# KLab/YAIK

Measured on AMD Instinct MI355X. Metric: Mpix/s tile encode (alpha reject + 7 gradient passes + 8x8 range quant), 8K RGBA, higher is better.
Workload: dtype u8/int32 (+f32 mode-selection sums)

## Files before the change

### yaik_amd/csrc/yk_api.hip

```cpp
#include "yk_common.h"
#ifdef YK_TEST_HOOKS
#include "../../include/yaik_hip_test.h"
#endif
#include <cstdio>
#include <cstring>
#include <utility>
#include <vector>

int yk_fail(yk_ctx* c, int code, const char* what, hipError_t e) {
    if (c && c->err.empty()) {
        c->err = what ? what : "error";
        if (e != hipSuccess) { c->err += ": "; c->err += hipGetErrorString(e); }
    }
    return code;
}

int yk_refuse(yk_ctx* c, int code, const char* what) {
    if (c) c->err = what ? what : "error";
    return code;
}

void yk_rebase(yk_ctx* c, int f) {
    const YkFrameStrides& fs = c->fs; auto& B = c->B;
    c->curFrame = f;
    for (int i = 0; i < 4; i++) c->plane[i] = B.plane[i] ? B.plane[i] + (size_t)f * fs.plane : nullptr;
    c->keep = B.keep + (size_t)f * fs.keep; c->bounds = B.bounds + (size_t)f * 16;
    for (int i = 0; i < 7; i++) c->bitmap[i] = B.bitmap[i] + (size_t)f * fs.bitmap[i];
    c->coverage = B.coverage + (size_t)f * fs.coverage; c->tileDef = B.tileDef + (size_t)f * fs.tileDef;
    c->tileCount = B.tileCount + (size_t)f * fs.tileCount; c->slots = B.slots + (size_t)f * fs.slots;
    c->blockSums = B.blockSums + (size_t)f * fs.blockN; c->blockCnt = B.blockCnt + (size_t)f * fs.blockN;
    c->totals = B.totals + (size_t)f * 8; c->defsOut = B.defsOut + (size_t)f * fs.defsOut; c->nibOut = B.nibOut + (size_t)f * fs.nibOut;
}

static void yk_input_changed(yk_ctx* c) {
    c->encoded = false; c->alphaDone = false; c->alphaFinished = false; c->avBatchValid = false; c->img.sb.valid = false; c->pal.valid = false;
    c->cornersReady = false; c->ppActive = false; c->ppLastBit = 0; c->previewFresh = false;
}

static void yk_encode_done(yk_ctx* c, int wantDst) {
    c->encoded = true; c->dstValid = wantDst != 0; c->img.sb.valid = false; c->pal.valid = false; c->cornersReady = false; c->ppActive = false;
    c->ppLastBit = 0; c->previewFresh = false; c->nextCornerPass = 0; c->r1Ready = false;
}

static void yk_free_image(yk_ctx* c) {
    c->img = YkImageBufs();
    { yk_ctx::Bases none = {}; for (int i = 0; i < 4; i++) none.plane[i] = c->B.plane[i]; c->B = none; }
    c->keep = nullptr; c->bounds = nullptr; for (int i = 0; i < 7; i++) c->bitmap[i] = nullptr;
    c->coverage = nullptr; c->tileDef = nullptr; c->tileCount = nullptr; c->slots = nullptr;
    c->blockSums = nullptr; c->blockCnt = nullptr; c->totals = nullptr; c->defsOut = nullptr; c->nibOut = nullptr;
    c->ppBitmapBytes = c->ppStreamBytes = 0; c->r1Ready = false; c->pixCacheValid = false;
    if (c->frameGraph) { (void)hipGraphExecDestroy(c->frameGraph); c->frameGraph = nullptr; }
    yk_input_changed(c);
}

static int yk_alloc_image_run(yk_ctx* c) {
    const size_t F = (size_t)c->nFrames;
    const size_t T8 = (size_t)c->tilesW * c->tilesH, MT = (size_t)c->mtW * c->mtH;
    auto& B = c->B; auto& M = c->img; YkFrameStrides& fs = c->fs; const hipStream_t s = c->stream;
    auto up = [](size_t n, size_t a) { return (n + a - 1) / a * a; };
    fs.keep = up(MT + 4, 16);
    YK_HIP(c, M.keep.alloc(s, fs.keep * F, 16));
    YK_HIP(c, M.bounds.alloc(s, 16 * F));
    {
        const size_t nUnits = (size_t)((c->fullW / 4 + 63) / 64) * c->mtH, nGroups = (nUnits + 63) / 64;
        YK_HIP(c, M.alphaUnitBox.alloc(s, (nUnits + nGroups) * F * 4, 16));
        YK_HIP(c, M.alphaArrive.alloc(s, (nGroups + 1) * F, 16));
        YK_HIP(c, hipMemset(M.alphaArrive, 0, (nGroups + 1) * F * sizeof(uint32_t) + 16));
    }
    static const int sh[7][2] = { {4,4},{4,3},{3,4},{3,3},{3,2},{2,3},{2,2} };
    size_t cur = 0, oBm[7], oBm0b, oCov, oInfo, oRun;
    auto place = [&](size_t bytesPerFrame) { const size_t o = cur; cur = up(cur + bytesPerFrame * F + 16, 256); return o; };
    for (int i = 0; i < 7; i++) {
        const int bx = (sh[i][0] == 2) ? 32 : 64, by = (sh[i][1] == 2) ? 32 : 64;
        const size_t bits = (size_t)((c->fullW + bx - 1) / bx) * ((c->h + by - 1) / by) * ((bx >> sh[i][0]) * (by >> sh[i][1]));
        c->bitmapBytes[i] = bits >> 3;
        fs.bitmap[i] = up(c->bitmapBytes[i] + 4, 16);
        oBm[i] = place(fs.bitmap[i]);
    }
    const size_t nB64 = (size_t)((c->fullW + 63) / 64) * ((c->h + 63) / 64);
    fs.bm0b = up(nB64 * 4, 16); oBm0b = place(fs.bm0b);
    fs.coverage = up(MT, 8); oCov = place(fs.coverage * sizeof(uint16_t));
    fs.tileInfo = up(T8, 2); oInfo = place(fs.tileInfo * sizeof(uint2));
    fs.runSums = up((T8 + 7) / 8, 4); oRun = place(fs.runSums * sizeof(uint32_t));
    if (cur >= ((size_t)1 << 32)) return yk_fail(c, YK_ERR_BAD_ARG, "image too large for 32-bit offsets into the small-output arena");
    YK_HIP(c, M.small.alloc(s, cur));
    YK_HIP(c, hipMemset(M.small, 0, cur));
    B.small = M.small;
    for (int i = 0; i < 7; i++) B.bitmap[i] = B.small + oBm[i];
    B.bm0b = B.small + oBm0b; B.coverage = reinterpret_cast<uint16_t*>(B.small + oCov);
    B.tileInfo = reinterpret_cast<uint2*>(B.small + oInfo); B.runSums = reinterpret_cast<uint32_t*>(B.small + oRun);
    fs.tileDef = 3 * T8; fs.tileCount = 3 * T8; fs.slots = 3 * T8 * YK_SLOT;
    YK_HIP(c, M.tileDef.alloc(s, fs.tileDef * F, 16));
    YK_HIP(c, M.tileCount.alloc(s, fs.tileCount * F, 16));
    YK_HIP(c, M.slots.alloc(s, fs.slots * F, 16));
    c->nScanBlocks = (int)((T8 + 1023) / 1024);
    fs.blockN = (size_t)c->nScanBlocks * 2;
    YK_HIP(c, M.blockSums.alloc(s, fs.blockN * F));
    YK_HIP(c, M.blockCnt.alloc(s, fs.blockN * F));
    YK_HIP(c, hipMemset(M.blockCnt, 0, fs.blockN * F * sizeof(uint32_t)));
    YK_HIP(c, M.totals.alloc(s, 8 * F));
    fs.defsOut = 3 * T8;
    YK_HIP(c, M.defsOut.alloc(s, fs.defsOut * F, 16));
    c->nibStride = T8 * YK_SLOT + 64;
    fs.nibOut = 3 * c->nibStride;
    YK_HIP(c, M.nibOut.alloc(s, fs.nibOut * F, 16));
    B.keep = M.keep; B.bounds = M.bounds; B.tileDef = M.tileDef; B.tileCount = M.tileCount; B.slots = M.slots;
    B.blockSums = M.blockSums; B.blockCnt = M.blockCnt; B.totals = M.totals; B.defsOut = M.defsOut; B.nibOut = M.nibOut;
    c->dstValid = false;
    yk_rebase(c, 0);
    return YK_OK;
}
static int yk_alloc_image(yk_ctx* c) {
    const int rc = yk_alloc_image_run(c);
    if (rc) yk_free_image(c);
    return rc;
}

static int yk_stage_fold(yk_ctx* c, int st) {
    for (int k = 0; k < c->stN[st]; k++) {
        float t = 0;
        YK_HIP(c, hipEventSynchronize(c->stEv[st][k][1]));
// ... 760 lines not shown
```

### yaik_amd/csrc/yk_common.h

```cpp
#pragma once
#include <hip/hip_runtime.h>
#include <stdint.h>
#include <stddef.h>
#include <memory>
#include <string>
#include <vector>
#include "../../include/yaik_hip.h"

#define YK_BLK      64
#define YK_LSTRIDE  68
#define YK_LROWS    65
#define YK_EV_RING  64
#define YK_SLOT     32
#define YK_NUM_STAGES 11
#define YK_STAGE_RING 16

struct YkFrameStrides {
    unsigned long long plane, keep, bitmap[7], coverage, tileDef, tileCount, slots, blockN, defsOut, nibOut;
    unsigned long long bm0b, tileInfo, runSums;
};

enum { YK_EVSET_ALPHA = 1, YK_EVSET_PACK = 2 };
enum { YK_EV_A0, YK_EV_E0, YK_EV_E1, YK_EV_P1, YK_EV_N };
struct YkEvRing {
// ... 34 lines not shown
    int ablate;
    const uint8_t* keep;
    const int32_t* bounds;
    uint8_t* bitmap[7];
    uint16_t* coverage;
    uint16_t* tileDef;
    uint8_t*  tileCount;
    uint8_t*  slots;
    uint32_t* blockCnt;
    int32_t*  dst[3];
    int tilesW, tilesH, mtW, mtH;
    int xBB64, yBB64, xBB32, yBB32;
    int nFrames;
    const uint8_t* qtab;
    uint8_t* small;
    uint32_t oBm[7], oBm0b, oCov, oInfo, oRun;
    uint4* pixCache;
    YkFrameStrides fs;
};

#define YK_SB_COUNTS 9
struct YkStreamRec { uint8_t* rgb[7]; uint8_t* pix; uint8_t* type; };
struct YkStreamsBatch {
    YkBuf<uint32_t> owner;
    YkBuf<uint32_t> cScratch;
    YkBuf<uint32_t> r1Scratch;
    YkBuf<uint32_t> counts;
    YkBuf<uint8_t> out;
    YkBuf<YkStreamRec> tab;
    std::vector<yk_frame_streams> table; bool valid = false;
    int what = 0;
};

struct YkPalette {
    YkBuf<uint8_t> scratch;
    YkBuf<uint8_t> out;
    YkBuf<uint32_t> carry;
    bool carryFresh = true;
    std::vector<uint8_t> segHost;
    std::vector<uint32_t> lenBase;
    int nSeg = 0; bool valid = false;
};

struct YkPaletteDec {
    YkBuf<uint8_t> scratch;
    YkBuf<uint8_t> out;
    YkBuf<uint8_t> stage;
    std::vector<size_t> slotOff, slotLen;
    std::vector<uint32_t> statusHost;
    size_t statusOff = 0;
    int nSeg = 0; bool valid = false;
};

struct YkImageBufs {
    YkBuf<uint8_t> keep; YkBuf<int32_t> bounds;
    YkBuf<int> alphaUnitBox;
    YkBuf<uint32_t> alphaArrive;
    YkBuf<uint8_t> small;
    YkBuf<uint16_t> tileDef; YkBuf<uint8_t> tileCount, slots;
    YkBuf<int32_t> dst[3];
    YkBuf<uint32_t> blockSums, blockCnt, totals;
    YkBuf<unsigned long long> exportSizes;
    YkBuf<uint16_t> defsOut; YkBuf<uint8_t> nibOut;
    YkBuf<uint32_t> latticeOwner; YkBuf<uint8_t> cornerStream; YkBuf<uint32_t> cornerScratch;
    YkBuf<uint32_t> cornerEdgeIdx;
    YkBuf<uint16_t> covCh;
    YkBuf<uint8_t> mapped3;
    YkBuf<uint32_t> ppBitmap; YkBuf<uint8_t> ppStream; YkBuf<uint32_t> ppScratch;
    YkBuf<int32_t> preview;
    YkBuf<uint8_t> r1Slots, r1Params; YkBuf<uint32_t> r1Cnt; YkBuf<uint8_t> r1Pix, r1Type;
    YkBuf<uint4> pixCache;
    YkStreamsBatch sb;
};

struct yk_ctx {
    int device = -1;
    int numCU = 256;
    const uint8_t* qtab = nullptr;
    hipStream_t ownStream = nullptr;
    hipStream_t stream = nullptr;
    std::string err;
    int fullW = 0, fullH = 0, nPlanes = 0, y0 = 0, h = 0, halo = 0;
    int tilesW = 0, tilesH = 0, mtW = 0, mtH = 0;
    int nFrames = 1, curFrame = 0;
    YkFrameStrides fs = {};
    struct Bases {
        const int32_t* plane[4]; uint8_t* keep; int32_t* bounds; uint8_t* bitmap[7]; uint16_t* coverage; uint16_t* tileDef; uint8_t* tileCount;
        uint8_t* slots; uint32_t* blockSums; uint32_t* blockCnt; uint32_t* totals; uint16_t* defsOut; uint8_t* nibOut;
        uint8_t* small;
        uint8_t* bm0b; uint2* tileInfo; uint32_t* runSums;
    } B = {};
    const int32_t* plane[4] = {nullptr, nullptr, nullptr, nullptr};
    int strideElems = 0;
    YkBuf<int32_t> ownedPlanes;
    YkBuf<uint8_t> pxStage;
    hipEvent_t evPixCopy = nullptr;
    uint8_t* keep = nullptr;
    int32_t* bounds = nullptr;
    int boundsOff = 8;
    bool alphaDone = false, alphaFinished = false;
    int32_t hostBounds[4] = {0, 0, 0, 0}; int hostDiscard = 1, hostHasChunk = 0;
    uint8_t* bitmap[7] = {}; size_t bitmapBytes[7] = {};
    uint16_t* coverage = nullptr;
    uint16_t* tileDef = nullptr; uint8_t* tileCount = nullptr; uint8_t* slots = nullptr;
    int32_t dstFill = -1; bool dstValid = false;
    uint32_t* blockSums = nullptr;
    uint32_t* blockCnt = nullptr;
    uint32_t* totals = nullptr;
    hipEvent_t evHandoff = nullptr;
    hipEvent_t fusedAfter = nullptr; std::shared_ptr<YkEvRing> fusedAfterRing;
// ... 94 lines not shown
```

### yaik_amd/csrc/yk_stages.hip

```cpp
#include "yk_common.h"
#ifdef YK_TEST_HOOKS
#include "../../include/yaik_hip_test.h"
#endif
#include "yk_device.h"

typedef int yk_i4 __attribute__((ext_vector_type(4)));
#ifndef YK_ALPHA_THREADS
#define YK_ALPHA_THREADS 256
#endif
#define YK_ALPHA_WAVES (YK_ALPHA_THREADS / 64)
#ifndef YK_ALPHA_ROWS
#define YK_ALPHA_ROWS 2
#endif
__global__ __launch_bounds__(YK_ALPHA_THREADS) void yk_alpha_kernel(const int32_t* __restrict__ alpha0, int strideElems, int w, int h, int y0,
                                                       uint8_t* __restrict__ keep0, int mtW, int mtH, int32_t* __restrict__ bounds,
                                                       int nFrames, unsigned long long planeStride, unsigned long long keepStride,
                                                       int* __restrict__ unitBox0, uint32_t* __restrict__ arrive0) {
    __shared__ int s_box[YK_ALPHA_WAVES][4];
    const int lane = threadIdx.x & 63, wv = threadIdx.x >> 6;
    const int vecPerRow = w >> 2;
    const int nSeg = (vecPerRow + YK_ALPHA_THREADS - 1) / YK_ALPHA_THREADS;
    const int nRowUnits = (mtH + YK_ALPHA_ROWS - 1) / YK_ALPHA_ROWS;
    const int nUnits = nSeg * nRowUnits, nGroups = (nUnits + 63) >> 6;
    for (long long uu = blockIdx.x; uu < (long long)nUnits * nFrames; uu += gridDim.x) {
        const int f = (int)(uu / nUnits), u = (int)(uu - (long long)f * nUnits);
        const int32_t* alpha = alpha0 + (size_t)f * planeStride;
        uint8_t* keep = keep0 + (size_t)f * keepStride;
        int* unitBox = unitBox0 + (size_t)f * (nUnits + nGroups) * 4;
        uint32_t* arrive = arrive0 + (size_t)f * (nGroups + 1);
        const int tyU = u / nSeg, seg = u - tyU * nSeg;
        const int xv = seg * YK_ALPHA_THREADS + (int)threadIdx.x;
        const bool inX = xv < vecPerRow;
        const bool tileLane = (lane & 3) == 0;
        const int tx = xv >> 2;
        int colLo = 0x7FFFFFFF, colHi = -1, rowLo = 0x7FFFFFFF, rowHi = -1;
        const int xvc = min(xv, vecPerRow - 1);
        int nzR[YK_ALPHA_ROWS];
        bool und[YK_ALPHA_ROWS];
        {
            yk_i4 p[YK_ALPHA_ROWS][2];
#pragma unroll
            for (int r = 0; r < YK_ALPHA_ROWS; r++) {
                const int yA = min((tyU * YK_ALPHA_ROWS + r) * 16, h - 1), yB = min(yA + 15, h - 1);
                p[r][0] = __builtin_nontemporal_load(reinterpret_cast<const yk_i4*>(alpha + (size_t)yA * strideElems + (size_t)xvc * 4));
                p[r][1] = __builtin_nontemporal_load(reinterpret_cast<const yk_i4*>(alpha + (size_t)yB * strideElems + (size_t)xvc * 4));
            }
            bool anyUnd = false;
#pragma unroll
            for (int r = 0; r < YK_ALPHA_ROWS; r++) {
                const bool on = inX && (tyU * YK_ALPHA_ROWS + r) * 16 < h;
                const yk_i4 o = p[r][0] | p[r][1];
                nzR[r] = on ? (o.x | o.y | o.z | o.w) : 0;
                const unsigned long long pb = __ballot(nzR[r] != 0);
                und[r] = on && ((pb >> (lane & ~3)) & 0xFULL) == 0;
                anyUnd |= und[r];
            }
            if (__ballot(anyUnd) != 0) {
                yk_i4 a[YK_ALPHA_ROWS][14];
#pragma unroll
                for (int r = 0; r < YK_ALPHA_ROWS; r++) {
                    const int ty = tyU * YK_ALPHA_ROWS + r;
                    const int32_t* col = alpha + (size_t)(ty * 16) * strideElems + (size_t)xv * 4;
#pragma unroll
                    for (int k = 0; k < 14; k++) {
                        a[r][k] = (yk_i4){0, 0, 0, 0};
                        if (und[r] && ty * 16 + 1 + k < h) a[r][k] = __builtin_nontemporal_load(reinterpret_cast<const yk_i4*>(col + (size_t)(1 + k) * strideElems));
                    }
                }
#pragma unroll
                for (int r = 0; r < YK_ALPHA_ROWS; r++)
#pragma unroll
                    for (int k = 0; k < 14; k++) nzR[r] |= a[r][k].x | a[r][k].y | a[r][k].z | a[r][k].w;
            }
        }
#pragma unroll
        for (int r = 0; r < YK_ALPHA_ROWS; r++) {
            const int ty = tyU * YK_ALPHA_ROWS + r;
            if (ty >= mtH) break;
            const int nz = nzR[r];
            const unsigned long long b = __ballot(nz != 0);
            const bool kept = ((b >> (lane & ~3)) & 0xFULL) != 0;
            if (tileLane && tx < mtW) keep[(size_t)ty * mtW + tx] = kept ? 1 : 0;
            const unsigned long long kb64 = __ballot(tileLane && kept && tx < mtW);
            if (kb64) {
                const int t0 = seg * (YK_ALPHA_THREADS / 4) + wv * 16;
                colLo = min(colLo, t0 + ((__ffsll((long long)kb64) - 1) >> 2));
                colHi = max(colHi, t0 + ((63 - __clzll((long long)kb64)) >> 2));
                rowLo = min(rowLo, ty); rowHi = max(rowHi, ty);
            }
        }
        if (lane == 0) { s_box[wv][0] = colLo; s_box[wv][1] = colHi; s_box[wv][2] = rowLo; s_box[wv][3] = rowHi; }
        __syncthreads();
        if (wv == 0) {
            unsigned long long* ub = reinterpret_cast<unsigned long long*>(unitBox);
            auto putBox = [&](const int slot, const int bx0, const int by0, const int bx1, const int by1) {
                __hip_atomic_store(&ub[slot * 2], ((unsigned long long)(uint32_t)by0 << 32) | (uint32_t)bx0, __ATOMIC_RELAXED, __HIP_MEMORY_SCOPE_AGENT);
                __hip_atomic_store(&ub[slot * 2 + 1], ((unsigned long long)(uint32_t)by1 << 32) | (uint32_t)bx1, __ATOMIC_RELAXED, __HIP_MEMORY_SCOPE_AGENT);
                __builtin_amdgcn_s_waitcnt(0);
            };
            auto foldBoxes = [&](const int first, const int n, int& x0, int& gy0, int& x1, int& gy1) {
                x0 = 9999999; gy0 = 9999999; x1 = -1; gy1 = -1;
                for (int k = lane; k < n; k += 64) {
                    const unsigned long long a = __hip_atomic_load(&ub[(first + k) * 2], __ATOMIC_RELAXED, __HIP_MEMORY_SCOPE_AGENT);
                    const unsigned long long bb = __hip_atomic_load(&ub[(first + k) * 2 + 1], __ATOMIC_RELAXED, __HIP_MEMORY_SCOPE_AGENT);
                    x0 = min(x0, (int)(uint32_t)a); gy0 = min(gy0, (int)(uint32_t)(a >> 32)); x1 = max(x1, (int)(uint32_t)bb); gy1 = max(gy1, (int)(uint32_t)(bb >> 32));
                }
#pragma unroll
                for (int d = 1; d < 64; d <<= 1) {
                    x0 = min(x0, __shfl_xor(x0, d)); x1 = max(x1, __shfl_xor(x1, d));
                    gy0 = min(gy0, __shfl_xor(gy0, d)); gy1 = max(gy1, __shfl_xor(gy1, d));
                }
            };
            const int g = u >> 6, inGroup = min(64, nUnits - (g << 6));
            uint32_t lastOfGroup = 0;
            if (lane == 0) {
                int lo = s_box[0][0], hi = s_box[0][1], rlo = s_box[0][2], rhi = s_box[0][3];
#pragma unroll
                for (int k = 1; k < YK_ALPHA_WAVES; k++) { lo = min(lo, s_box[k][0]); hi = max(hi, s_box[k][1]); rlo = min(rlo, s_box[k][2]); rhi = max(rhi, s_box[k][3]); }
                const bool any = hi >= 0;
                putBox(u, any ? lo * 16 : 9999999, any ? y0 + rlo * 16 : 9999999, any ? hi * 16 + 16 : -1, any ? y0 + rhi * 16 + 16 : -1);
                lastOfGroup = __hip_atomic_fetch_add(&arrive[g], 1u, __ATOMIC_RELAXED, __HIP_MEMORY_SCOPE_AGENT) == (uint32_t)inGroup - 1u ? 1u : 0u;
            }
            if (__builtin_amdgcn_readfirstlane((int)lastOfGroup)) {
                int x0, gy0, x1, gy1;
                foldBoxes(g << 6, inGroup, x0, gy0, x1, gy1);
                uint32_t lastOfFrame = 0;
                if (lane == 0) {
                    putBox(nUnits + g, x0, gy0, x1, gy1);
                    arrive[g] = 0u;
                    lastOfFrame = __hip_atomic_fetch_add(&arrive[nGroups], 1u, __ATOMIC_RELAXED, __HIP_MEMORY_SCOPE_AGENT) == (uint32_t)nGroups - 1u ? 1u : 0u;
                }
                if (__builtin_amdgcn_readfirstlane((int)lastOfFrame)) {
                    foldBoxes(nUnits, nGroups, x0, gy0, x1, gy1);
                    if (lane == 0) { int32_t* acc = bounds + (size_t)f * 16 + 8; acc[0] = x0; acc[1] = gy0; acc[2] = x1; acc[3] = gy1; arrive[nGroups] = 0u; }
                }
            }
        }
        if (uu + gridDim.x < (long long)nUnits * nFrames) __syncthreads();
    }
}

__global__ void yk_alpha_publish_kernel(int32_t* __restrict__ bounds, int srcOff, int fullW, int fullH) {
    bounds += (size_t)blockIdx.x * 16;
    const int b0 = bounds[srcOff], b1 = bounds[srcOff + 1], b2 = bounds[srcOff + 2], b3 = bounds[srcOff + 3];
    bounds[0] = b0; bounds[1] = b1; bounds[2] = b2; bounds[3] = b3;
    bounds[4] = (b0 == 0 && b1 == 0 && b2 == fullW && b3 == fullH) ? 1 : 0;
}

#define YK_SCAN_TILE 1024

__global__ __launch_bounds__(1024) void yk_scan1_kernel(const uint8_t* __restrict__ tileCount, size_t T8, uint32_t* __restrict__ blockCnt) {
    __shared__ uint32_t s_tmp[32];
    const size_t i = (size_t)blockIdx.x * YK_SCAN_TILE + threadIdx.x;
    const uint32_t c = (i < T8) ? tileCount[i] : 0;
    uint32_t tot2, totN;
    yk_block_exscan(c ? 1u : 0u, s_tmp, &tot2);
    yk_block_exscan(c, s_tmp, &totN);
    if (threadIdx.x == 0) { blockCnt[(size_t)blockIdx.x * 2] = totN; blockCnt[(size_t)blockIdx.x * 2 + 1] = tot2; }
}

__device__ __forceinline__ void yk_scan2_body(uint32_t* __restrict__ blockCnt, uint32_t* __restrict__ blockSums, int nBlocks, uint32_t* __restrict__ totals, uint32_t* s_tmp) {
    uint32_t baseN = 0, baseD = 0;
    for (int start = 0; start < nBlocks; start += 1024) {
        const int i = start + threadIdx.x;
        const uint32_t n = i < nBlocks ? blockCnt[i * 2] : 0, d = i < nBlocks ? blockCnt[i * 2 + 1] : 0;
        uint32_t totN, totD;
        const uint32_t en = yk_block_exscan(n, s_tmp, &totN);
        const uint32_t ed = yk_block_exscan(d, s_tmp, &totD);
        if (i < nBlocks) {
            blockSums[i * 2] = baseN + en; blockSums[i * 2 + 1] = baseD + ed;
            blockCnt[i * 2] = 0; blockCnt[i * 2 + 1] = 0;
        }
        baseN += totN; baseD += totD;
    }
    if (threadIdx.x < 3) { totals[threadIdx.x * 2] = baseD; totals[threadIdx.x * 2 + 1] = baseN; }
}
__global__ __launch_bounds__(1024) void yk_scan2_kernel(uint32_t* __restrict__ blockCnt, uint32_t* __restrict__ blockSums, int nBlocks,
                                                        uint32_t* __restrict__ totals, unsigned long long blockNStride) {
    __shared__ uint32_t s_tmp[32];
    yk_scan2_body(blockCnt + (size_t)blockIdx.x * blockNStride, blockSums + (size_t)blockIdx.x * blockNStride, nBlocks, totals + (size_t)blockIdx.x * 8, s_tmp);
}

__global__ __launch_bounds__(1024) void yk_scan1r_kernel(const uint32_t* __restrict__ runSums, unsigned long long runStride, int nRuns,
                                                         uint32_t* __restrict__ blockCnt, unsigned long long blockNStride, int nBlocks,
                                                         const uint8_t* __restrict__ bm0b, unsigned long long bm0bStride, uint8_t* __restrict__ bitmap0,
                                                         unsigned long long bitmap0Stride, int nB64) {
    const size_t f = blockIdx.y;
    const int g = (int)blockIdx.x * 1024 + (int)threadIdx.x;
    if (runSums) {
        const uint4* rs4 = reinterpret_cast<const uint4*>(runSums + f * runStride);
        const int n4 = (nRuns + 3) >> 2;
// ... 56 lines not shown
#pragma unroll
    for (int j = 0; j < 4; j++) { w[j] = mine; mine += c[j] | (c[j] ? 0x10000u : 0u); }
    uint32_t incl = mine;
#pragma unroll
    for (int d = 1; d < 64; d <<= 1) { const uint32_t o = __shfl_up(incl, d); if (lane >= d) incl += o; }
    if (lane == 63) s_wave[wave] = incl;
    __syncthreads();
    uint32_t front = incl - mine;
#pragma unroll
    for (int k = 0; k < 3; k++) if (k < wave) front += s_wave[k];
    uint32_t baseN, baseD;
    if (blockCnt) {
        baseN = (uint32_t)s_pre; baseD = (uint32_t)(s_pre >> 32);
        if (blockIdx.x == (unsigned)nBlocks - 1 && threadIdx.x < 3) {
            const uint2 v = reinterpret_cast<const uint2*>(blockCnt)[nBlocks - 1];
            totals[threadIdx.x * 2] = baseD + v.y; totals[threadIdx.x * 2 + 1] = baseN + v.x;
        }
    } else { baseN = blockSums[(size_t)blockIdx.x * 2]; baseD = blockSums[(size_t)blockIdx.x * 2 + 1]; }
#pragma unroll
    for (int j = 0; j < 4; j++) {
        const uint32_t e = front + w[j], en = e & 0xFFFFu, ed = e >> 16;
        s_off[threadIdx.x * 4 + j] = (baseN + en) >> 1;
        s_cnt[threadIdx.x * 4 + j] = (uint8_t)c[j];
        if (c[j]) { defsOut[baseD + ed] = (uint16_t)d01[j]; defsOut[T8 + baseD + ed] = (uint16_t)(d01[j] >> 16); defsOut[2 * T8 + baseD + ed] = (uint16_t)d2[j]; }
    }
    __syncthreads();
    const int half = threadIdx.x & 1;
#pragma unroll
    for (int p = 0; p < 3; p++) {
        uint8_t* out = reinterpret_cast<uint8_t*>(nibOut + (size_t)p * nibStrideWords);
#pragma unroll
        for (int it = 0; it < 8; it++) {
            const int t = it * 128 + (threadIdx.x >> 1);
            const size_t ti = i0 + t;
            const int left = (s_cnt[t] >> 1) - half * 16;
            const uint8_t* src = slots + ((size_t)p * T8 + ti) * YK_SLOT + half * 16;
            uint8_t* dst = out + s_off[t] + half * 16;
            if (left >= 16) { const uint4 v = *reinterpret_cast<const uint4*>(src); *reinterpret_cast<YkPiece16*>(dst) = YkPiece16{v.x, v.y, v.z, v.w}; }
            else if (left >= 8) *reinterpret_cast<uint2*>(dst) = *reinterpret_cast<const uint2*>(src);
        }
    }
}

static int (*g_crossCheckLauncher)(hipStream_t, const YkEncodeParams*) = nullptr;
#ifdef YK_TEST_HOOKS
extern "C" int yk_set_cross_check_launcher(void* fn) { g_crossCheckLauncher = reinterpret_cast<int (*)(hipStream_t, const YkEncodeParams*)>(fn); return YK_OK; }
#endif

int yk_launch_alpha(yk_ctx* c, bool batch) {
    const int F = batch ? c->nFrames : 1;
    uint8_t* keep = batch ? c->B.keep : c->keep;
    int32_t* bounds = batch ? c->B.bounds : c->bounds;
    const int32_t* alpha = batch ? c->B.plane[3] : c->plane[3];
    const int nSeg = (c->fullW / 4 + YK_ALPHA_THREADS - 1) / YK_ALPHA_THREADS;
    const long long nUnits = (long long)nSeg * ((c->mtH + YK_ALPHA_ROWS - 1) / YK_ALPHA_ROWS) * F;
    const long long maxWG = 4096LL * (256 / YK_ALPHA_THREADS);
    hipLaunchKernelGGL(yk_alpha_kernel, dim3((unsigned)(nUnits < maxWG ? nUnits : maxWG)), dim3(YK_ALPHA_THREADS), 0, c->stream, alpha, c->strideElems, c->fullW, c->h, c->y0,
                       keep, c->mtW, c->mtH, bounds, F, (unsigned long long)c->fs.plane, (unsigned long long)c->fs.keep, c->img.alphaUnitBox, c->img.alphaArrive);
    YK_HIP(c, hipGetLastError());
    c->boundsOff = 8;
    return YK_OK;
}

int yk_launch_alpha_finish(yk_ctx* c, const int32_t* globalBBox) {
    if (globalBBox) {
        int32_t b[5] = { globalBBox[0], globalBBox[1], globalBBox[2], globalBBox[3], 0 };
        b[4] = (b[0] == 0 && b[1] == 0 && b[2] == c->fullW && b[3] == c->fullH) ? 1 : 0;
        YK_HIP(c, hipMemcpyAsync(c->bounds, b, sizeof b, hipMemcpyHostToDevice, c->stream));
        c->boundsOff = 0;
    }
    return YK_OK;
}

int yk_launch_encode(yk_ctx* c, int rejectFactor, int mode3BitOnly, int wantDst, bool batch) {
    YkEncodeParams P;
    for (int i = 0; i < 4; i++) P.plane[i] = batch ? c->B.plane[i] : c->plane[i];
    P.strideElems = c->strideElems; P.w = c->fullW; P.h = c->h; P.hAvail = c->h + c->halo; P.y0 = c->y0; P.fullH = c->fullH;
    P.rejectFactor = rejectFactor; P.startMode = mode3BitOnly ? 3 : 0; P.wantDst = wantDst; P.ablate = c->ablate;
    P.keep = (c->nPlanes == 4) ? (batch ? c->B.keep : c->keep) : nullptr;
    P.bounds = (c->nPlanes == 4) ? (batch ? c->B.bounds : c->bounds) + c->boundsOff : nullptr;
    for (int i = 0; i < 7; i++) P.bitmap[i] = batch ? c->B.bitmap[i] : c->bitmap[i];
    P.coverage = batch ? c->B.coverage : c->coverage; P.tileDef = batch ? c->B.tileDef : c->tileDef;
    P.tileCount = batch ? c->B.tileCount : c->tileCount; P.slots = batch ? c->B.slots : c->slots;
    P.blockCnt = c->kernelVersion == 2 ? (batch ? c->B.blockCnt : c->blockCnt) : nullptr;
    for (int i = 0; i < 3; i++) P.dst[i] = c->img.dst[i];
    P.tilesW = c->tilesW; P.tilesH = c->tilesH; P.mtW = c->mtW; P.mtH = c->mtH;
    P.xBB64 = (c->fullW + 63) / 64; P.yBB64 = (c->h + 63) / 64; P.xBB32 = (c->fullW + 31) / 32; P.yBB32 = (c->h + 31) / 32;
    P.nFrames = batch ? c->nFrames : 1; P.fs = c->fs;
    P.qtab = c->qtab;
    P.small = c->B.small;
    for (int i = 0; i < 7; i++) P.oBm[i] = (uint32_t)(c->B.bitmap[i] - c->B.small);
    P.oBm0b = (uint32_t)(c->B.bm0b - c->B.small); P.oCov = (uint32_t)(reinterpret_cast<uint8_t*>(c->B.coverage) - c->B.small);
    P.oInfo = (uint32_t)(reinterpret_cast<uint8_t*>(c->B.tileInfo) - c->B.small); P.oRun = (uint32_t)(reinterpret_cast<uint8_t*>(c->B.runSums) - c->B.small);
    if (!batch && c->curFrame) {
        for (int i = 0; i < 7; i++) P.oBm[i] += (uint32_t)(c->curFrame * c->fs.bitmap[i]);
        P.oBm0b += (uint32_t)(c->curFrame * c->fs.bm0b); P.oCov += (uint32_t)(c->curFrame * c->fs.coverage * 2);
        P.oInfo += (uint32_t)(c->curFrame * c->fs.tileInfo * 8); P.oRun += (uint32_t)(c->curFrame * c->fs.runSums * 4);
    }
    P.pixCache = nullptr; c->pixCacheValid = false;
    if (c->pixCacheOn && !batch && c->kernelVersion == 2 && c->nFrames == 1) {
        if (!c->img.pixCache) YK_HIP(c, c->img.pixCache.alloc(c->stream, (size_t)P.xBB64 * 64 * ((size_t)(c->h + 15) / 16 * 16) / 4, 4096));
        P.pixCache = c->img.pixCache; c->pixCacheValid = true;
    }
    if (c->kernelVersion == 2) return yk_launch_encode2(c, P);
    if (batch) return yk_fail(c, YK_ERR_STATE, "batches need kernel version 2");
    if (c->nPlanes == 4) {
        hipLaunchKernelGGL(yk_alpha_publish_kernel, dim3(1), dim3(1), 0, c->stream, c->bounds, c->boundsOff, c->fullW, c->fullH);
        P.bounds = c->bounds;
    }
    if (!g_crossCheckLauncher) return yk_fail(c, YK_ERR_STATE, "kernel version 1 is not part of this library: register it with yk_set_cross_check_launcher");
    if (g_crossCheckLauncher(c->stream, &P) != 0) return yk_fail(c, YK_ERR_HIP, "cross-check kernel launch", hipGetLastError());
// ... 90 lines not shown
```

Before: 223,600.

## Split alpha reject into per-wave units plus separate bounding-box fold kernel

Replaces the persistent-grid alpha kernel, which used atomic arrival counters and a last-block fold, with a one-wave-per-unit kernel that writes per-unit boxes, followed by a small per-frame reduction kernel. Each wave now handles 4 tile rows with a lazy two-rows-at-a-time interior scan for undecided rows, and blocks are 3 waves with an occupancy hint. This removes cross-workgroup atomics, the __syncthreads and the arrive buffer. In exchange it adds an extra kernel launch and a read-back of the unit boxes. A profiling summary script is also added.

```diff
diff --git a/profiles/alpha_stream/summarize.py b/profiles/alpha_stream/summarize.py
--- /dev/null
+++ b/profiles/alpha_stream/summarize.py
@@ -0,0 +1,63 @@
+import collections, csv, glob, os, runpy, statistics, sys
+
+mode, d = sys.argv[1], sys.argv[2]
+S, E = (lambda r: int(r["Start_Timestamp"])), (lambda r: int(r["End_Timestamp"]))
+
+
+def kernel_rows(pattern):
+    rows = []
+    for f in glob.glob(f"{d}/**/*kernel_trace.csv", recursive=True):
+        rows += [r for r in csv.DictReader(open(f)) if pattern(r["Kernel_Name"])]
+    rows.sort(key=S)
+    return rows
+
+
+if mode == "timeline":
+    sys.argv = [os.path.join(os.path.dirname(os.path.abspath(__file__)), "..", "event_chain", "summarize.py"), "timeline", d]
+    runpy.run_path(sys.argv[0], run_name="__main__")
+    rows = kernel_rows(lambda n: "yk_alpha" in n or "encode2" in n)
+    fused = [r for r in rows if "encode2" in r["Kernel_Name"]]
+    has_fold = any("yk_alpha_box_kernel" in r["Kernel_Name"] for r in rows)
+    stages, open_ = [], {}
+    for r in rows:
+        q = r.get("Queue_Id", "?")
+        if "yk_alpha_kernel" in r["Kernel_Name"]:
+            if has_fold:
+                open_.setdefault(q, S(r))
+            else:
+                stages.append((S(r), E(r)))
+        elif "yk_alpha_box_kernel" in r["Kernel_Name"] and q in open_:
+            stages.append((open_.pop(q), E(r)))
+    lo, hi = S(fused[len(fused) // 4]), S(fused[len(fused) * 3 // 4])
+    rel, into, dur = [], [], []
+    for s0, e0 in stages:
+        if not lo <= s0 <= hi:
+            continue
+        beside = [r for r in fused if S(r) <= s0 < E(r)]
+        if not beside:
+            continue
+        rel.append((e0 - E(beside[0])) / 1e3); into.append((e0 - S(beside[0])) / 1e3); dur.append((e0 - s0) / 1e3)
+    print(f"alpha stage ({'alpha + fold' if has_fold else 'alpha kernel'}), {len(rel)} frames: ends {statistics.mean(rel):+.1f} us relative to the end of the other frame's fused kernel "
+          f"(min {min(rel):+.1f}, max {max(rel):+.1f}), {statistics.mean(into):.1f} us after its start; start to end {statistics.mean(dur):.1f} us")
+    sys.exit(0)
+reps, planes = int(sys.argv[3]), sys.argv[4:]
+per = reps + 3
+if mode == "trace":
+    alpha, fold = kernel_rows(lambda n: "yk_alpha_kernel" in n), kernel_rows(lambda n: "yk_alpha_box_kernel" in n)
+    assert len(alpha) == per * len(planes) and len(fold) in (0, len(alpha)), (len(alpha), len(fold), per, planes)
+    for i, p in enumerate(planes):
+        sel = range(i * per + 2, i * per + 2 + reps)
+        us = [((E(fold[k]) if fold else E(alpha[k])) - S(alpha[k])) / 1e3 for k in sel]
+        extra = f"  fold kernel median {statistics.median((E(fold[k]) - S(fold[k])) / 1e3 for k in sel):4.1f} us" if fold else ""
+        print(f"plane {p}: alpha stage min {min(us):6.1f} us  median {statistics.median(us):6.1f} us  max {max(us):6.1f} us  ({reps} launches){extra}")
+else:
+    acc = collections.defaultdict(float)
+    for f in glob.glob(f"{d}/**/*counter_collection.csv", recursive=True):
+        for r in csv.DictReader(open(f)):
+            if "yk_alpha_kernel" in r["Kernel_Name"] and r["Counter_Name"] == "FETCH_SIZE":
+                acc[int(r["Dispatch_Id"])] += float(r["Counter_Value"])
+    ids = sorted(acc)
+    assert len(ids) == per * len(planes), (len(ids), per, planes)
+    for i, p in enumerate(planes):
+        kb = acc[ids[i * per + per - 2]]
+        print(f"plane {p}: yk_alpha_kernel FETCH_SIZE {kb:.0f} KB -> {kb * 1024 * 2 / 1e6:.1f} MB (x1024, x2 on gfx950)")
diff --git a/yaik_amd/csrc/yk_api.hip b/yaik_amd/csrc/yk_api.hip
--- a/yaik_amd/csrc/yk_api.hip
+++ b/yaik_amd/csrc/yk_api.hip
@@ -61,12 +61,7 @@
     fs.keep = up(MT + 4, 16);
     YK_HIP(c, M.keep.alloc(s, fs.keep * F, 16));
     YK_HIP(c, M.bounds.alloc(s, 16 * F));
-    {
-        const size_t nUnits = (size_t)((c->fullW / 4 + 63) / 64) * c->mtH, nGroups = (nUnits + 63) / 64;
-        YK_HIP(c, M.alphaUnitBox.alloc(s, (nUnits + nGroups) * F * 4, 16));
-        YK_HIP(c, M.alphaArrive.alloc(s, (nGroups + 1) * F, 16));
-        YK_HIP(c, hipMemset(M.alphaArrive, 0, (nGroups + 1) * F * sizeof(uint32_t) + 16));
-    }
+    YK_HIP(c, M.alphaUnitBox.alloc(s, yk_alpha_units(c->fullW, c->mtH) * F * 4, 16));
     static const int sh[7][2] = { {4,4},{4,3},{3,4},{3,3},{3,2},{2,3},{2,2} };
     size_t cur = 0, oBm[7], oBm0b, oCov, oInfo, oRun;
     auto place = [&](size_t bytesPerFrame) { const size_t o = cur; cur = up(cur + bytesPerFrame * F + 16, 256); return o; };
diff --git a/yaik_amd/csrc/yk_common.h b/yaik_amd/csrc/yk_common.h
--- a/yaik_amd/csrc/yk_common.h
+++ b/yaik_amd/csrc/yk_common.h
@@ -110,10 +110,14 @@
     int nSeg = 0; bool valid = false;
 };
 
+#ifndef YK_ALPHA_R
+#define YK_ALPHA_R 4
+#endif
+static inline size_t yk_alpha_units(int fullW, int mtH) { return (size_t)((fullW / 4 + 63) / 64) * (size_t)((mtH + YK_ALPHA_R - 1) / YK_ALPHA_R); }
+
 struct YkImageBufs {
     YkBuf<uint8_t> keep; YkBuf<int32_t> bounds;
     YkBuf<int> alphaUnitBox;
-    YkBuf<uint32_t> alphaArrive;
     YkBuf<uint8_t> small;
     YkBuf<uint16_t> tileDef; YkBuf<uint8_t> tileCount, slots;
     YkBuf<int32_t> dst[3];
diff --git a/yaik_amd/csrc/yk_stages.hip b/yaik_amd/csrc/yk_stages.hip
--- a/yaik_amd/csrc/yk_stages.hip
+++ b/yaik_amd/csrc/yk_stages.hip
@@ -5,138 +5,115 @@
 #include "yk_device.h"
 
 typedef int yk_i4 __attribute__((ext_vector_type(4)));
-#ifndef YK_ALPHA_THREADS
-#define YK_ALPHA_THREADS 256
+#ifndef YK_ALPHA_WAVES
+#define YK_ALPHA_WAVES 3
 #endif
-#define YK_ALPHA_WAVES (YK_ALPHA_THREADS / 64)
-#ifndef YK_ALPHA_ROWS
-#define YK_ALPHA_ROWS 2
-#endif
-__global__ __launch_bounds__(YK_ALPHA_THREADS) void yk_alpha_kernel(const int32_t* __restrict__ alpha0, int strideElems, int w, int h, int y0,
-                                                       uint8_t* __restrict__ keep0, int mtW, int mtH, int32_t* __restrict__ bounds,
-                                                       int nFrames, unsigned long long planeStride, unsigned long long keepStride,
-                                                       int* __restrict__ unitBox0, uint32_t* __restrict__ arrive0) {
-    __shared__ int s_box[YK_ALPHA_WAVES][4];
+__global__ __launch_bounds__(64 * YK_ALPHA_WAVES, 4) void yk_alpha_kernel(const int32_t* __restrict__ alpha0, int strideElems, int w, int h, int y0,
+                                                      uint8_t* __restrict__ keep0, int mtW, int mtH, unsigned long long planeStride,
+                                                      unsigned long long keepStride, yk_i4* __restrict__ unitBox0, unsigned total) {
+    const int lane = threadIdx.x & 63;
+    const int vecPerRow = w >> 2;
+    const int nSeg = (vecPerRow + 63) >> 6;
+    const int nUnits = nSeg * ((mtH + YK_ALPHA_R - 1) / YK_ALPHA_R);
+    const unsigned uu = blockIdx.x * YK_ALPHA_WAVES + (threadIdx.x >> 6);
+    if (uu >= total) return;
+    const int f = (int)(uu / (unsigned)nUnits), u = (int)(uu - (unsigned)f * (unsigned)nUnits);
+    const int32_t* alpha = alpha0 + (size_t)f * planeStride;
+    uint8_t* keep = keep0 + (size_t)f * keepStride;
+    const int tyU = u / nSeg, seg = u - tyU * nSeg, ty0 = tyU * YK_ALPHA_R;
+    const int xv = seg * 64 + lane;
+    const bool inX = xv < vecPerRow;
+    const bool tileLane = (lane & 3) == 0;
+    const int tx = xv >> 2;
+    const int xvc = min(xv, vecPerRow - 1);
+    uint32_t nzBits = 0, undBits = 0, rowsLeft = 0;
+    {
+        yk_i4 p[YK_ALPHA_R][2];
+#pragma unroll
+        for (int r = 0; r < YK_ALPHA_R; r++) {
+            const int yA = min((ty0 + r) * 16, h - 1), yB = min(yA + 15, h - 1);
+            p[r][0] = __builtin_nontemporal_load(reinterpret_cast<const yk_i4*>(alpha + (size_t)yA * strideElems + (size_t)xvc * 4));
+            p[r][1] = __builtin_nontemporal_load(reinterpret_cast<const yk_i4*>(alpha + (size_t)yB * strideElems + (size_t)xvc * 4));
+        }
+#pragma unroll
+        for (int r = 0; r < YK_ALPHA_R; r++) {
+            const bool on = inX && (ty0 + r) * 16 < h;
+            const yk_i4 o = p[r][0] | p[r][1];
+            const bool nz = ((o.x | o.y | o.z | o.w) != 0) & on;
+            const unsigned long long pb = __ballot(nz);
+            const bool und = on && ((pb >> (lane & ~3)) & 0xFULL) == 0;
+            nzBits |= (nz ? 1u : 0u) << r; undBits |= (und ? 1u : 0u) << r;
+            if (__ballot(und) != 0) rowsLeft |= 1u << r;
+        }
+    }
+    while (rowsLeft) {
+        const int rA = __ffs((int)rowsLeft) - 1; rowsLeft &= rowsLeft - 1;
+        const bool two = rowsLeft != 0;
+        const int rB = two ? __ffs((int)rowsLeft) - 1 : rA; rowsLeft &= rowsLeft - 1;
+        yk_i4 a[2][14];
+#pragma unroll
+        for (int j = 0; j < 2; j++) {
+            const int r = j ? rB : rA, ty = ty0 + r;
+            const bool und = (j == 0 || two) && ((undBits >> r) & 1u) != 0;
+            const int32_t* col = alpha + (size_t)(ty * 16) * strideElems + (size_t)xv * 4;
+#pragma unroll
+            for (int k = 0; k < 14; k++) {
+                a[j][k] = (yk_i4){0, 0, 0, 0};
+                if (und && ty * 16 + 1 + k < h) a[j][k] = __builtin_nontemporal_load(reinterpret_cast<const yk_i4*>(col + (size_t)(1 + k) * strideElems));
+            }
+        }
+#pragma unroll
+        for (int j = 0; j < 2; j++) {
+            int m = 0;
+#pragma unroll
+            for (int k = 0; k < 14; k++) m |= a[j][k].x | a[j][k].y | a[j][k].z | a[j][k].w;
+            nzBits |= (m != 0 ? 1u : 0u) << (j ? rB : rA);
+        }
+    }
+    int colLo = 0x7FFFFFFF, colHi = -1, rowLo = 0x7FFFFFFF, rowHi = -1;
+#pragma unroll
+    for (int r = 0; r < YK_ALPHA_R; r++) {
+        const int ty = ty0 + r;
+        if (ty >= mtH) break;
+        const unsigned long long b = __ballot(((nzBits >> r) & 1u) != 0);
+        const bool kept = ((b >> (lane & ~3)) & 0xFULL) != 0;
+        if (tileLane && tx < mtW) keep[(size_t)ty * mtW + tx] = kept ? 1 : 0;
+        const unsigned long long kb64 = __ballot(tileLane && kept && tx < mtW);
+        if (kb64) {
+            colLo = min(colLo, seg * 16 + ((__ffsll((long long)kb64) - 1) >> 2));
+            colHi = max(colHi, seg * 16 + ((63 - __clzll((long long)kb64)) >> 2));
+            rowLo = min(rowLo, ty); rowHi = max(rowHi, ty);
+        }
+    }
+    if (lane == 0) {
+        const bool any = colHi >= 0;
+        unitBox0[(size_t)f * nUnits + u] = any ? (yk_i4){colLo * 16, y0 + rowLo * 16, colHi * 16 + 16, y0 + rowHi * 16 + 16} : (yk_i4){9999999, 9999999, -1, -1};
+    }
+}
+
+__global__ __launch_bounds__(256) void yk_alpha_box_kernel(const yk_i4* __restrict__ unitBox0, int nUnits, int32_t* __restrict__ bounds) {
+    __shared__ yk_i4 s_box[4];
     const int lane = threadIdx.x & 63, wv = threadIdx.x >> 6;
-    const int vecPerRow = w >> 2;
-    const int nSeg = (vecPerRow + YK_ALPHA_THREADS - 1) / YK_ALPHA_THREADS;
-    const int nRowUnits = (mtH + YK_ALPHA_ROWS - 1) / YK_ALPHA_ROWS;
-    const int nUnits = nSeg * nRowUnits, nGroups = (nUnits + 63) >> 6;
-    for (long long uu = blockIdx.x; uu < (long long)nUnits * nFrames; uu += gridDim.x) {
-        const int f = (int)(uu / nUnits), u = (int)(uu - (long long)f * nUnits);
-        const int32_t* alpha = alpha0 + (size_t)f * planeStride;
-        uint8_t* keep = keep0 + (size_t)f * keepStride;
-        int* unitBox = unitBox0 + (size_t)f * (nUnits + nGroups) * 4;
-        uint32_t* arrive = arrive0 + (size_t)f * (nGroups + 1);
-        const int tyU = u / nSeg, seg = u - tyU * nSeg;
-        const int xv = seg * YK_ALPHA_THREADS + (int)threadIdx.x;
-        const bool inX = xv < vecPerRow;
-        const bool tileLane = (lane & 3) == 0;
-        const int tx = xv >> 2;
-        int colLo = 0x7FFFFFFF, colHi = -1, rowLo = 0x7FFFFFFF, rowHi = -1;
-        const int xvc = min(xv, vecPerRow - 1);
-        int nzR[YK_ALPHA_ROWS];
-        bool und[YK_ALPHA_ROWS];
-        {
-            yk_i4 p[YK_ALPHA_ROWS][2];
-#pragma unroll
-            for (int r = 0; r < YK_ALPHA_ROWS; r++) {
-                const int yA = min((tyU * YK_ALPHA_ROWS + r) * 16, h - 1), yB = min(yA + 15, h - 1);
-                p[r][0] = __builtin_nontemporal_load(reinterpret_cast<const yk_i4*>(alpha + (size_t)yA * strideElems + (size_t)xvc * 4));
-                p[r][1] = __builtin_nontemporal_load(reinterpret_cast<const yk_i4*>(alpha + (size_t)yB * strideElems + (size_t)xvc * 4));
-            }
-            bool anyUnd = false;
-#pragma unroll
-            for (int r = 0; r < YK_ALPHA_ROWS; r++) {
-                const bool on = inX && (tyU * YK_ALPHA_ROWS + r) * 16 < h;
-                const yk_i4 o = p[r][0] | p[r][1];
-                nzR[r] = on ? (o.x | o.y | o.z | o.w) : 0;
-                const unsigned long long pb = __ballot(nzR[r] != 0);
-                und[r] = on && ((pb >> (lane & ~3)) & 0xFULL) == 0;
-                anyUnd |= und[r];
-            }
-            if (__ballot(anyUnd) != 0) {
-                yk_i4 a[YK_ALPHA_ROWS][14];
-#pragma unroll
-                for (int r = 0; r < YK_ALPHA_ROWS; r++) {
-                    const int ty = tyU * YK_ALPHA_ROWS + r;
-                    const int32_t* col = alpha + (size_t)(ty * 16) * strideElems + (size_t)xv * 4;
-#pragma unroll
-                    for (int k = 0; k < 14; k++) {
-                        a[r][k] = (yk_i4){0, 0, 0, 0};
-                        if (und[r] && ty * 16 + 1 + k < h) a[r][k] = __builtin_nontemporal_load(reinterpret_cast<const yk_i4*>(col + (size_t)(1 + k) * strideElems));
-                    }
-                }
-#pragma unroll
-                for (int r = 0; r < YK_ALPHA_ROWS; r++)
-#pragma unroll
-                    for (int k = 0; k < 14; k++) nzR[r] |= a[r][k].x | a[r][k].y | a[r][k].z | a[r][k].w;
-            }
-        }
-#pragma unroll
-        for (int r = 0; r < YK_ALPHA_ROWS; r++) {
-            const int ty = tyU * YK_ALPHA_ROWS + r;
-            if (ty >= mtH) break;
-            const int nz = nzR[r];
-            const unsigned long long b = __ballot(nz != 0);
-            const bool kept = ((b >> (lane & ~3)) & 0xFULL) != 0;
-            if (tileLane && tx < mtW) keep[(size_t)ty * mtW + tx] = kept ? 1 : 0;
-            const unsigned long long kb64 = __ballot(tileLane && kept && tx < mtW);
-            if (kb64) {
-                const int t0 = seg * (YK_ALPHA_THREADS / 4) + wv * 16;
-                colLo = min(colLo, t0 + ((__ffsll((long long)kb64) - 1) >> 2));
-                colHi = max(colHi, t0 + ((63 - __clzll((long long)kb64)) >> 2));
-                rowLo = min(rowLo, ty); rowHi = max(rowHi, ty);
-            }
-        }
-        if (lane == 0) { s_box[wv][0] = colLo; s_box[wv][1] = colHi; s_box[wv][2] = rowLo; s_box[wv][3] = rowHi; }
-        __syncthreads();
-        if (wv == 0) {
-            unsigned long long* ub = reinterpret_cast<unsigned long long*>(unitBox);
-            auto putBox = [&](const int slot, const int bx0, const int by0, const int bx1, const int by1) {
-                __hip_atomic_store(&ub[slot * 2], ((unsigned long long)(uint32_t)by0 << 32) | (uint32_t)bx0, __ATOMIC_RELAXED, __HIP_MEMORY_SCOPE_AGENT);
-                __hip_atomic_store(&ub[slot * 2 + 1], ((unsigned long long)(uint32_t)by1 << 32) | (uint32_t)bx1, __ATOMIC_RELAXED, __HIP_MEMORY_SCOPE_AGENT);
-                __builtin_amdgcn_s_waitcnt(0);
-            };
-            auto foldBoxes = [&](const int first, const int n, int& x0, int& gy0, int& x1, int& gy1) {
-                x0 = 9999999; gy0 = 9999999; x1 = -1; gy1 = -1;
-                for (int k = lane; k < n; k += 64) {
-                    const unsigned long long a = __hip_atomic_load(&ub[(first + k) * 2], __ATOMIC_RELAXED, __HIP_MEMORY_SCOPE_AGENT);
-                    const unsigned long long bb = __hip_atomic_load(&ub[(first + k) * 2 + 1], __ATOMIC_RELAXED, __HIP_MEMORY_SCOPE_AGENT);
-                    x0 = min(x0, (int)(uint32_t)a); gy0 = min(gy0, (int)(uint32_t)(a >> 32)); x1 = max(x1, (int)(uint32_t)bb); gy1 = max(gy1, (int)(uint32_t)(bb >> 32));
-                }
-#pragma unroll
-                for (int d = 1; d < 64; d <<= 1) {
-                    x0 = min(x0, __shfl_xor(x0, d)); x1 = max(x1, __shfl_xor(x1, d));
-                    gy0 = min(gy0, __shfl_xor(gy0, d)); gy1 = max(gy1, __shfl_xor(gy1, d));
-                }
-            };
-            const int g = u >> 6, inGroup = min(64, nUnits - (g << 6));
-            uint32_t lastOfGroup = 0;
-            if (lane == 0) {
-                int lo = s_box[0][0], hi = s_box[0][1], rlo = s_box[0][2], rhi = s_box[0][3];
-#pragma unroll
-                for (int k = 1; k < YK_ALPHA_WAVES; k++) { lo = min(lo, s_box[k][0]); hi = max(hi, s_box[k][1]); rlo = min(rlo, s_box[k][2]); rhi = max(rhi, s_box[k][3]); }
-                const bool any = hi >= 0;
-                putBox(u, any ? lo * 16 : 9999999, any ? y0 + rlo * 16 : 9999999, any ? hi * 16 + 16 : -1, any ? y0 + rhi * 16 + 16 : -1);
-                lastOfGroup = __hip_atomic_fetch_add(&arrive[g], 1u, __ATOMIC_RELAXED, __HIP_MEMORY_SCOPE_AGENT) == (uint32_t)inGroup - 1u ? 1u : 0u;
-            }
-            if (__builtin_amdgcn_readfirstlane((int)lastOfGroup)) {
-                int x0, gy0, x1, gy1;
-                foldBoxes(g << 6, inGroup, x0, gy0, x1, gy1);
-                uint32_t lastOfFrame = 0;
-                if (lane == 0) {
-                    putBox(nUnits + g, x0, gy0, x1, gy1);
-                    arrive[g] = 0u;
-                    lastOfFrame = __hip_atomic_fetch_add(&arrive[nGroups], 1u, __ATOMIC_RELAXED, __HIP_MEMORY_SCOPE_AGENT) == (uint32_t)nGroups - 1u ? 1u : 0u;
-                }
-                if (__builtin_amdgcn_readfirstlane((int)lastOfFrame)) {
-                    foldBoxes(nUnits, nGroups, x0, gy0, x1, gy1);
-                    if (lane == 0) { int32_t* acc = bounds + (size_t)f * 16 + 8; acc[0] = x0; acc[1] = gy0; acc[2] = x1; acc[3] = gy1; arrive[nGroups] = 0u; }
-                }
-            }
-        }
-        if (uu + gridDim.x < (long long)nUnits * nFrames) __syncthreads();
+    const yk_i4* ub = unitBox0 + (size_t)blockIdx.x * nUnits;
+    int x0 = 9999999, gy0 = 9999999, x1 = -1, gy1 = -1;
+    for (int base = 0; base < nUnits; base += 256 * 16) {
+        yk_i4 v[16];
+#pragma unroll
+        for (int j = 0; j < 16; j++) v[j] = ub[min(base + j * 256 + (int)threadIdx.x, nUnits - 1)];
+#pragma unroll
+        for (int j = 0; j < 16; j++) { x0 = min(x0, v[j].x); gy0 = min(gy0, v[j].y); x1 = max(x1, v[j].z); gy1 = max(gy1, v[j].w); }
+    }
+#pragma unroll
+    for (int d = 1; d < 64; d <<= 1) {
+        x0 = min(x0, __shfl_xor(x0, d)); x1 = max(x1, __shfl_xor(x1, d));
+        gy0 = min(gy0, __shfl_xor(gy0, d)); gy1 = max(gy1, __shfl_xor(gy1, d));
+    }
+    if (lane == 0) s_box[wv] = (yk_i4){x0, gy0, x1, gy1};
+    __syncthreads();
+    if (threadIdx.x == 0) {
+#pragma unroll
+        for (int k = 1; k < 4; k++) { x0 = min(x0, s_box[k].x); gy0 = min(gy0, s_box[k].y); x1 = max(x1, s_box[k].z); gy1 = max(gy1, s_box[k].w); }
+        *reinterpret_cast<yk_i4*>(bounds + (size_t)blockIdx.x * 16 + 8) = (yk_i4){x0, gy0, x1, gy1};
     }
 }
 
@@ -299,11 +276,12 @@
     uint8_t* keep = batch ? c->B.keep : c->keep;
     int32_t* bounds = batch ? c->B.bounds : c->bounds;
     const int32_t* alpha = batch ? c->B.plane[3] : c->plane[3];
-    const int nSeg = (c->fullW / 4 + YK_ALPHA_THREADS - 1) / YK_ALPHA_THREADS;
-    const long long nUnits = (long long)nSeg * ((c->mtH + YK_ALPHA_ROWS - 1) / YK_ALPHA_ROWS) * F;
-    const long long maxWG = 4096LL * (256 / YK_ALPHA_THREADS);
-    hipLaunchKernelGGL(yk_alpha_kernel, dim3((unsigned)(nUnits < maxWG ? nUnits : maxWG)), dim3(YK_ALPHA_THREADS), 0, c->stream, alpha, c->strideElems, c->fullW, c->h, c->y0,
-                       keep, c->mtW, c->mtH, bounds, F, (unsigned long long)c->fs.plane, (unsigned long long)c->fs.keep, c->img.alphaUnitBox, c->img.alphaArrive);
+    const long long nUnits = (long long)yk_alpha_units(c->fullW, c->mtH);
+    if (nUnits * F > 0x7FFFFFFFLL) return yk_fail(c, YK_ERR_BAD_ARG, "too many alpha work units for one launch");
+    yk_i4* unitBox = reinterpret_cast<yk_i4*>(static_cast<int*>(c->img.alphaUnitBox));
+    hipLaunchKernelGGL(yk_alpha_kernel, dim3((unsigned)((nUnits * F + YK_ALPHA_WAVES - 1) / YK_ALPHA_WAVES)), dim3(64 * YK_ALPHA_WAVES), 0, c->stream, alpha, c->strideElems,
+                       c->fullW, c->h, c->y0, keep, c->mtW, c->mtH, (unsigned long long)c->fs.plane, (unsigned long long)c->fs.keep, unitBox, (unsigned)(nUnits * F));
+    hipLaunchKernelGGL(yk_alpha_box_kernel, dim3((unsigned)F), dim3(256), 0, c->stream, unitBox, (int)nUnits, bounds);
     YK_HIP(c, hipGetLastError());
     c->boundsOff = 8;
     return YK_OK;
```

After: 226,600, median of 6. 1.01x the previous value.
